# earthspecies/avex

Measured on AMD Instinct MI355X. Metric: clips/s (10 s @ 16 kHz) embedding extraction, BEATs-base, higher is better.
Workload: dtype f16; 1 GPU; BEATs-base (12L/768/3072/12H, 90.7 M params, synthetic weights), batch 256 x 10 s @ 16 kHz per GPU, wav resident in HBM -> mean-pooled 768-d embedding; global_batch=256, samples_per_clip=160000, parallelism=dp1, world_size=1, inputs=avex_amd.synth.noise_clips(seed=0), keyed by global clip index, chunk_clips=256, streams=1, residual_stream=half, layernorm_fold=True

## Files before the change

### avex_amd/_capi.py

```python
from __future__ import annotations

import ctypes as C
import os
from typing import Optional

HERE = os.path.dirname(os.path.abspath(__file__))
LIB_PATH = os.environ.get("AVEX_AMD_LIB") or os.path.join(HERE, "lib", "libavexhip.so")

F16, BF16 = 0, 1
DTYPE_NAMES = {"f16": F16, "fp16": F16, "float16": F16, "bf16": BF16, "bfloat16": BF16}


class AvexHipError(RuntimeError):
    """Raised for any failure of the HIP extension (missing library, no GPU, bad arguments)."""


class FbankConfig(C.Structure):
    _fields_ = [("win_length", C.c_int32), ("hop_length", C.c_int32), ("n_mels", C.c_int32),
                ("input_scale", C.c_float), ("preemph", C.c_float), ("remove_dc", C.c_int32),
                ("log_floor", C.c_float), ("norm_mean", C.c_float), ("norm_div", C.c_float)]


class MelspecConfig(C.Structure):
    _fields_ = [("n_fft", C.c_int32), ("hop_length", C.c_int32), ("win_length", C.c_int32), ("n_mels", C.c_int32),
# ... 126 lines not shown
    "avexhip_fbank_forward_padded": (C.c_int, [_P, _P, C.c_int, C.c_int64, C.c_int64, _P, C.c_int, _P, _P]),
    "avexhip_fbank_forward_patches": (C.c_int, [_P, _P, C.c_int, C.c_int64, C.c_int64, _P, C.c_int, C.c_int, _P, C.c_int, _P]),
    "avexhip_token_embed_ln": (C.c_int, [_P, _P, _P, _P, _P, C.c_float, C.c_int, C.c_int, C.c_int, _P, _P, C.c_int, _P]),
    "avexhip_cast_f32_to_half": (C.c_int, [_P, _P, C.c_int64, C.c_int, _P]),
    "avexhip_cast_half_to_f32": (C.c_int, [_P, _P, C.c_int64, C.c_int, _P]),
    "avexhip_gemm": (C.c_int, [C.POINTER(GemmArgs), C.c_int, _P]),
    "avexhip_pool_reduce": (C.c_int, [_P, C.c_int, C.c_int, C.c_int, _P, C.c_int64, _P]),
    "avexhip_pool_reduce_mode": (C.c_int, [_P, C.c_int, C.c_int, C.c_int, _P, C.c_int64, C.c_int, _P]),
    "avexhip_ln_rowstats": (C.c_int, [_P, C.c_int, C.c_int, C.c_float, _P, _P]),
    "avexhip_layernorm": (C.c_int, [_P, _P, C.c_int64, _P, _P, C.c_float, C.c_int, C.c_int, _P, C.c_int64, _P,
                                    C.c_int64, C.c_int, _P]),
    "avexhip_attention": (C.c_int, [_P, C.c_int, C.c_int, C.c_int, _P, _P, _P, _P, _P, _P, C.c_int, _P]),
    "avexhip_attention_hd": (C.c_int, [_P, C.c_int, C.c_int, C.c_int, C.c_int, _P, _P, C.c_int, _P]),
    "avexhip_posconv_pack": (C.c_int, [_P, _P, C.c_int, C.c_int, C.c_int, _P, C.c_int, _P]),
    "avexhip_posconv": (C.c_int, [_P, _P, _P, _P, C.c_int, C.c_int, C.c_int, C.c_int, C.c_int, _P, _P, C.c_int, _P]),
    "avexhip_mean_pool": (C.c_int, [_P, C.c_int, C.c_int, C.c_int, _P, _P]),
    "avexhip_rel_bucket": (C.c_int, [C.c_int, C.c_int, C.c_int]),
    "avexhip_beats_create": (_P, [C.POINTER(BeatsConfig), C.POINTER(Tensor), C.c_int]),
    "avexhip_beats_destroy": (None, [_P]),
    "avexhip_beats_num_tokens": (C.c_int, [_P, C.c_int64]),
    "avexhip_beats_workspace_bytes": (C.c_size_t, [_P, C.c_int, C.c_int64]),
    "avexhip_beats_forward": (C.c_int, [_P, _P, C.c_int, C.c_int64, C.c_int64, _P, C.c_uint32, C.POINTER(_P),
                                        C.c_int, _P, _P, _P, C.c_size_t, _P]),
    "avexhip_beats_forward_fbank": (C.c_int, [_P, _P, C.c_int, C.c_int, _P, C.c_uint32, C.POINTER(_P), C.c_int,
                                              _P, _P, _P, C.c_size_t, _P]),
    "avexhip_beats_graph_capture": (_P, [_P, _P, C.c_int, C.c_int64, C.c_int64, _P, C.c_uint32, C.POINTER(_P),
                                         C.c_int, _P, _P, _P, C.c_size_t, _P]),
    "avexhip_beats_graph_launch": (C.c_int, [_P, _P]),
    "avexhip_beats_graph_nodes": (C.c_int, [_P]),
    "avexhip_beats_graph_destroy": (None, [_P]),
# ... 131 lines not shown
```

### avex_amd/csrc/api.cpp

```cpp
#include <math.h>
#include <stdarg.h>
#include <stdlib.h>

#include <map>
#include <mutex>
#include <utility>
#include <string>
#include <vector>

#include "common.h"
#include "handle_core.h"

static thread_local char g_err[1024] = "";

void avexhip_set_error(const char* fmt, ...) {
    va_list ap;
    va_start(ap, fmt);
    vsnprintf(g_err, sizeof(g_err), fmt, ap);
    va_end(ap);
}

extern "C" const char* avexhip_last_error(void) { return g_err; }
extern "C" int avexhip_abi_version(void) { return AVEXHIP_ABI_VERSION; }
extern "C" int avexhip_device_count(void) {
// ... 75 lines not shown
extern "C" int avexhip_layernorm(const float* in, const void* in_half, int64_t ld_in, const float* w, const float* b,
                                 float eps, int M, int C, float* out_f32, int64_t ldo, void* out_half, int64_t ldh,
                                 int dtype, void* stream) {
    return avx::layernorm(in, in_half, ld_in, w, b, eps, M, C, out_f32, ldo, out_half, ldh, dtype, (hipStream_t)stream);
}

extern "C" int avexhip_attention(const void* qkv, int B, int T, int H, const float* bias_tab, const float* grep_w,
                                 const float* grep_b, const float* grep_a, const uint8_t* key_pad, void* out,
                                 int dtype, void* stream) {
    return avx::attention(qkv, B, T, H, bias_tab, grep_w, grep_b, grep_a, key_pad, out, dtype, (hipStream_t)stream);
}

extern "C" int avexhip_posconv_pack(const float* g, const float* v, int E, int groups, int K, void* w_packed,
                                    int dtype, void* stream) {
    return avx::posconv_pack(g, v, E, groups, K, w_packed, dtype, (hipStream_t)stream);
}

extern "C" int avexhip_posconv(const void* x_half, const float* x_f32, const void* w_packed, const float* bias, int B,
                               int T, int E, int groups, int K, float* out_f32, void* out_half, int dtype, void* stream) {
    return avx::posconv(x_half, x_f32, w_packed, bias, B, T, E, groups, K, out_f32, out_half, dtype, (hipStream_t)stream);
}

extern "C" int avexhip_token_embed_ln(const void* patches_half, const float* pos, const float* cls, const float* ln_w, const float* ln_b, float eps,
                                      int B, int n_patches, int C, void* out_half, float* out_f32, int dtype, void* stream) {
    return avx::token_embed_ln(patches_half, pos, cls, ln_w, ln_b, eps, B, n_patches, C, out_half, out_f32, dtype, (hipStream_t)stream);
}

extern "C" int avexhip_mean_pool(const float* in, int B, int T, int C, float* out, void* stream) {
    return avx::mean_pool(in, B, T, C, nullptr, out, (hipStream_t)stream);
}
// ... 80 lines not shown
    float* lnE_w = nullptr; float* lnE_b = nullptr;
    std::vector<Layer> layers;
    std::vector<float> rel_table;
    struct BiasTab { float* ptr; hipEvent_t ready; hipStream_t stream; bool done; };
    float* d_rel_table = nullptr;
    int* d_bucket_lut = nullptr;
    int lut_maxd = 0;
    char* bias_arena = nullptr; size_t bias_arena_bytes = 0, bias_arena_used = 0;
    std::map<int, BiasTab> bias_tabs;
    std::mutex bias_mu;

    CoreCfg core() const {
        CoreCfg c;
        c.E = E; c.F = F; c.H = H; c.L = L; c.alpha = alpha; c.eps = 1e-5f; c.hook_site = 0; c.fast = fast; c.fold = ln_fold;
        c.fold_min_rows = ln_fold_min_rows; c.batch_invariant = batch_invariant; c.act = act; c.glu = glu; c.hidden_shift = hidden_shift; c.pre_ln = pre_ln; c.final_ln_w = lnE_w; c.final_ln_b = lnE_b;
        return c;
    }
    ~avexhip_beats() override {
        for (auto& kv : bias_tabs) if (kv.second.ready) (void)hipEventDestroy(kv.second.ready);
        if (bias_arena) (void)hipFree(bias_arena);
        if (d_rel_table) (void)hipFree(d_rel_table);
        if (d_bucket_lut) (void)hipFree(d_bucket_lut);
        if (fb) avexhip_fbank_plan_destroy(fb);
        for (int i = 0; i < 3; ++i) { if (side[i]) (void)hipStreamDestroy(side[i]); if (ev_join[i]) (void)hipEventDestroy(ev_join[i]); }
        if (ev_fork) (void)hipEventDestroy(ev_fork);
    }
};

namespace {

const avxh::LayerNames BEATS_NAMES = {nullptr, "encoder.layers.%d.self_attn.q_proj", "encoder.layers.%d.self_attn.k_proj", "encoder.layers.%d.self_attn.v_proj",
                                      "encoder.layers.%d.self_attn.out_proj", "encoder.layers.%d.self_attn_layer_norm", "encoder.layers.%d.fc1",
// ... 244 lines not shown
        const int lane_id = li;
        hipStream_t cs = lane_id == 0 ? s : h->side[lane_id - 1];
        const Ws w = carve(h, (char*)workspace + (size_t)lane_id * need.total, chunk, Tt);
        const uint8_t* pad = frame_pad ? frame_pad + (size_t)c0 * Tt : nullptr;
        const double Md = (double)M;
        if (h->fe_in_lane) RC(frontend(c0, Bc, w, cs));

        const bool fast = h->fast;
        float* x32 = w.core.x;
        float* pre32 = fast ? nullptr : w.core.pre;
        void* preh = fast ? w.core.preh : nullptr;
        const bool hook0 = (hook_mask & 1u) != 0;
        avx::GemmArgs g;
        memset(&g, 0, sizeof(g)); g.ovf = h->d_ovf;
        g.A = w.patches; g.lda = P * P; g.W = h->w_patch; g.ldw = P * P; g.M = M; g.N = D; g.K = P * P; g.bias = h->b_patch;
        if (fast) { g.out_half = w.h0; g.ldh = D; } else { g.out_f32 = w.f0; g.ldo = D; }
        prof.begin("gemm.patch_embed", 2.0 * Md * D * P * P);
        RC(avx::gemm(g, dt, cs));
        prof.end();
        prof.begin("layernorm", 0.0);
        if (h->w_post) {
            RC(avx::layernorm(fast ? nullptr : w.f0, fast ? w.h0 : nullptr, D, h->ln0_w, h->ln0_b, 1e-5f, M, D, nullptr, D, w.h0, D, dt, cs));
        } else {
            RC(avx::layernorm(fast ? nullptr : w.f0, fast ? w.h0 : nullptr, D, h->ln0_w, h->ln0_b, 1e-5f, M, D, fast ? nullptr : x32, E, w.core.xh, E, dt, cs));
            RC(avx::zero_rows(fast ? nullptr : x32, E, w.core.xh, E, M, E, pad, cs));
        }
        prof.end();
        if (h->w_post) {
            memset(&g, 0, sizeof(g)); g.ovf = h->d_ovf;
            g.A = w.h0; g.lda = D; g.W = h->w_post; g.ldw = D; g.M = M; g.N = E; g.K = D; g.bias = h->b_post;
            g.out_half = w.core.xh; g.ldh = E; g.row_zero = pad;
            if (!fast || hook0) { g.out_f32 = x32; g.ldo = E; }
            prof.begin("gemm.post_extract_proj", 2.0 * Md * E * D);
            RC(avx::gemm(g, dt, cs));
            prof.end();
        }
        if (hook0 && h->w_post) {
            if (hook_pooled) RC(avx::agg_pool(x32, Bc, Tt, E, hook_pooled, hook_out[0] + (size_t)c0 * E, cs));
            else AVX_HIP_CHECK(hipMemcpyAsync(hook_out[0] + (size_t)c0 * Tt * E, x32, sizeof(float) * (size_t)M * E, hipMemcpyDeviceToDevice, cs));
        }
        prof.begin("posconv", 2.0 * Md * E * (E / h->cfg.conv_pos_groups) * h->cfg.conv_pos);
        RC(avx::posconv(w.core.xh, fast ? nullptr : x32, h->w_pc, h->b_pc, Bc, Tt, E, h->cfg.conv_pos_groups, h->cfg.conv_pos, pre32, preh, dt, cs));
        prof.end();
        if (!h->pre_ln) {
            prof.begin("layernorm", 0.0);
            RC(avx::layernorm(pre32, preh, E, h->lnE_w, h->lnE_b, 1e-5f, M, E, fast ? nullptr : x32, E, w.core.xh, E, dt, cs));
            prof.end();
        }

        CoreIo io;
        io.Bc = Bc; io.Tt = Tt; io.c0 = (size_t)c0; io.bias_tab = bias_tab; io.pad = pad; io.hook_mask = hook_mask; io.hook_bit0 = 1;
        io.hook_out = hook_out; io.hook_pooled = hook_pooled; io.features_out = features_out; io.pooled_out = pooled_out;
        RC(avxh::run_layers(h, h->core(), h->layers, w.core, io, prof, cs));
        if (L == 0) {
            if (features_out || pooled_out) {
                float* xo = features_out ? features_out + (size_t)c0 * Tt * E : x32;
                RC(avx::layernorm(pre32, preh, E, h->lnE_w, h->lnE_b, 1e-5f, M, E, xo, E, nullptr, E, dt, cs));
                if (pooled_out) RC(avx::mean_pool(xo, Bc, Tt, E, nullptr, pooled_out + (size_t)c0 * E, cs));
            }
        }
    }
    if (lanes > 1) {
        for (int i = 0; i + 1 < lanes; ++i) {
            if (h->ev_join[i]) (void)hipEventDestroy(h->ev_join[i]);
            AVX_HIP_CHECK(hipEventCreateWithFlags(&h->ev_join[i], hipEventDisableTiming));
            AVX_HIP_CHECK(hipEventRecord(h->ev_join[i], h->side[i]));
            AVX_HIP_CHECK(hipStreamWaitEvent(s, h->ev_join[i], 0));
// ... 244 lines not shown
```

### avex_amd/csrc/common.h

```cpp
#pragma once
#include <hip/hip_runtime.h>
#include <stdint.h>
#include <stdio.h>
#include <string.h>

#include "../../include/avexhip.h"

typedef _Float16 f16x8 __attribute__((ext_vector_type(8)));
typedef _Float16 f16x4 __attribute__((ext_vector_type(4)));
typedef __bf16 bf16x8 __attribute__((ext_vector_type(8)));
typedef __bf16 bf16x4 __attribute__((ext_vector_type(4)));
typedef float f32x4 __attribute__((ext_vector_type(4)));
typedef float f32x16 __attribute__((ext_vector_type(16)));

template <typename T> struct Half;
template <> struct Half<_Float16> {
    typedef f16x8 v8;
    typedef f16x4 v4;
    static __device__ __forceinline__ _Float16 from(float x) {
        const float lo = x < -65504.0f ? -65504.0f : x;
        return (_Float16)(lo > 65504.0f ? 65504.0f : lo);
    }
    static __device__ __forceinline__ _Float16 from_hw(float x) { return (_Float16)x; }
};
// ... 279 lines not shown
int gemm(const GemmArgs& a, int dtype, hipStream_t s);
int nhwc_to_nchw(const float* in, int64_t ld, int B, int HW, int C, const float* scale, const float* shift, float* out, hipStream_t s);
int64_t mbconv_front_tiles(int H, int W, int k, int stride, int kin);
int dwconv_parts(const void* in, int B, int H, int W, int Cp, int k, int stride, const float* w, const float* bias, void* out, float* part, size_t part_bytes,
                 int64_t* rows, int dtype, hipStream_t s);
int64_t dwconv_lds_tiles(int H, int W, int k, int stride);
int dwconv_lds_parts(const void* in, int B, int H, int W, int Cp, int k, int stride, const float* w, const float* bias, void* out, float* part,
                     size_t part_bytes, int64_t* rows, int dtype, hipStream_t s);
int se_from_parts(const float* part, int64_t rows, int B, int64_t hw, int C, int Cp, int Cs, const float* w1, const float* b1, const float* w2t,
                  const float* b2, float* scale, void* x, int dtype, hipStream_t s);
int mbconv_front(const void* in, int B, int H, int W, int ld_in, int kin, const void* w_exp, int ldw, const float* b_exp, int k, int stride,
                 const float* w_dw, const float* b_dw, int cp_exp, void* out, float* pool, float* part, size_t part_bytes, unsigned int* ovf,
                 int dtype, hipStream_t s);
int pool_reduce(const float* part, int B, int T, int N, float* out, int64_t ldo, hipStream_t s, int mode = 0);
int agg_pool(const float* in, int B, int T, int C, int mode, float* out, hipStream_t s);
int ln_rowstats(const float* stats, int M, int nseg, float eps, float* rows, hipStream_t s);
int bias_toeplitz(const float* rel_table, const int* lut, int maxd, int T, int H, float* out, hipStream_t s);
int lnr_fold(const float* gamma, const float* beta, const float* bias, float alpha, int N, float* ga, float* bb, hipStream_t s);
int layernorm(const float* in, const void* in_half, int64_t ld_in, const float* w, const float* b, float eps, int M,
              int C, float* out_f32, int64_t ldo, void* out_half, int64_t ldh, int dtype, hipStream_t s);
int cast_to_half(const float* in, void* out, int64_t n, int dtype, hipStream_t s, unsigned int* ovf = nullptr);
int row_sum_half(const void* w, int N, int K, float* out, int dtype, hipStream_t s);
int cast_to_f32(const void* in, float* out, int64_t n, int dtype, hipStream_t s);
int mean_pool(const float* in, int B, int T, int C, const uint8_t* frame_pad, float* out, hipStream_t s);
int token_embed_ln(const void* patches, const float* pos, const float* cls, const float* w, const float* b, float eps, int B, int Tp, int C,
                   void* out_half, float* out_f32, int dtype, hipStream_t s);
int glu_swish(const void* in, int64_t M, int F, void* out, unsigned int* ovf, int dtype, hipStream_t s);
int zero_rows(float* x32, int64_t ld32, void* x_half, int64_t ldh, int M, int C, const uint8_t* pad, hipStream_t s);
int layernorm_pool(const void* in_half, int64_t ld_in, const float* w, const float* b, float eps, int B, int T, int C, float* out, int dtype,
                   hipStream_t s);
bool gemm_streams(int M, int N);
bool gemm_post_ln_ok(const GemmArgs& a);
int attention(const void* qkv, int B, int T, int H, const float* bias_tab, const float* grep_w,
              const float* grep_b, const float* grep_a, const uint8_t* key_pad, void* out, int dtype,
              hipStream_t s, int q_log2e = 0);
int attention16(const void* qkv, int B, int T, int H, const float* bias_tab, const float* grep_w, const float* grep_b, const float* grep_a,
                const uint8_t* key_pad, void* out, int dtype, int q_log2e, int n_wg, hipStream_t s);
int attention_hd(const void* qkv, int B, int T, int H, int head_dim, const uint8_t* key_pad, void* out, int dtype, hipStream_t s, int q_log2e = 0);
int posconv_pack(const float* g, const float* v, int E, int groups, int K, void* w_packed, int dtype,
                 hipStream_t s);
int posconv(const void* x_half, const float* x_f32, const void* w_packed, const float* bias, int B, int T,
            int E, int groups, int K, float* out_f32, void* out_half, int dtype, hipStream_t s);

struct FbankDev {
    int win, hop, n_mels;
    float input_scale, preemph, log_floor, norm_mean, norm_div;
    int remove_dc;
    const float* window;
    const float2* twiddle;
    const int* mel_start;
    const int* mel_len;
    const int* mel_off;
    const float* mel_w;
};
int fbank(const FbankDev& fb, const float* wav, int B, int64_t T, int64_t stride, int frames,
          float* out_f32, void* out_patch, int patch, int dtype, hipStream_t s, const float* clip_offset = nullptr,
          int out_frames = 0);
// ... 5 lines not shown
```

### avex_amd/csrc/elementwise.hip

```cpp
#include "common.h"

namespace {

template <typename T>
__global__ void cast_to_half_kernel(const float* __restrict__ in, T* __restrict__ out, int64_t n, unsigned int* __restrict__ ovf) {
    int64_t i = ((int64_t)blockIdx.x * blockDim.x + threadIdx.x) * 4;
    const int64_t stride = (int64_t)gridDim.x * blockDim.x * 4;
    float ovf_mx = 0.f;
    for (; i + 3 < n; i += stride) {
        const f32x4 v = *(const f32x4*)(in + i);
        ovf_see4<T>(ovf_mx, v);
        typename Half<T>::v4 h;
        h[0] = Half<T>::from(v[0]); h[1] = Half<T>::from(v[1]);
        h[2] = Half<T>::from(v[2]); h[3] = Half<T>::from(v[3]);
        *(typename Half<T>::v4*)(out + i) = h;
    }
    if (blockIdx.x == 0 && threadIdx.x < (n & 3)) {
        const int64_t j = (n & ~(int64_t)3) + threadIdx.x;
        ovf_see<T>(ovf_mx, in[j], 0.f);
        out[j] = Half<T>::from(in[j]);
    }
    ovf_commit<T>(ovf, ovf_mx);
}

// ... 354 lines not shown
        *(v8*)(out + m * F + f) = o;
    }
    ovf_commit<T>(ovf, mx);
}

template <typename T>
__global__ __launch_bounds__(256) void row_sum_half_kernel(const T* __restrict__ w, int N, int K, float* __restrict__ out) {
    const int row = blockIdx.x * 4 + (threadIdx.x >> 6), lane = threadIdx.x & 63;
    if (row >= N) return;
    float s = 0.f;
    for (int k = lane; k < K; k += 64) s += (float)w[(int64_t)row * K + k];
    s = wave_sum(s);
    if (lane == 0) out[row] = s;
}

__global__ __launch_bounds__(256) void ln_rowstats_kernel(const float* __restrict__ stats, int M, int nseg, float eps, float* __restrict__ rows) {
    const int m = blockIdx.x * 256 + threadIdx.x;
    if (m >= M) return;
    const f32x4* src = (const f32x4*)(stats + (int64_t)m * nseg * 2);
    float s1 = 0.f, s2 = 0.f;
    for (int q = 0; q < (nseg >> 1); ++q) { const f32x4 v = src[q]; s1 += v[0] + v[2]; s2 += v[1] + v[3]; }
    const float inv = 1.0f / (float)(64 * nseg);
    const float mu = s1 * inv;
    const float var = fmaxf(__builtin_fmaf(-mu, mu, s2 * inv), 0.f);
    const float rstd = __builtin_amdgcn_rsqf(var + eps);
    ((float2*)rows)[m] = make_float2(rstd, -mu * rstd);
}

__global__ __launch_bounds__(256) void pool_reduce_kernel(const float* __restrict__ part, int B, int T, int N, float* __restrict__ out, int64_t ldo, int mode) {
    const int n = blockIdx.x * 256 + threadIdx.x, b = blockIdx.y;
    if (n >= N) return;
    const int64_t r0 = (int64_t)b * T, r1 = r0 + T - 1;
    float acc = mode == 1 ? -__builtin_inff() : 0.f;
    for (int64_t rb = r0 >> 6; rb <= (r1 >> 6); ++rb) {
        const int64_t first_clip = (rb * 64) / T;
        const float v = part[(rb * 2 + (first_clip == b ? 0 : 1)) * N + n];
        acc = mode == 1 ? fmaxf(acc, v) : acc + v;
// ... 37 lines not shown

int bias_toeplitz(const float* rel_table, const int* lut, int maxd, int T, int H, float* out, hipStream_t s) {
    const int n = H * (2 * T - 1);
    hipLaunchKernelGGL(bias_toeplitz_kernel, dim3((unsigned)((n + 255) / 256)), dim3(256), 0, s, rel_table, lut, maxd, T, H, out);
    AVX_LAUNCH_CHECK();
    return AVEXHIP_OK;
}

int lnr_fold(const float* gamma, const float* beta, const float* bias, float alpha, int N, float* ga, float* bb, hipStream_t s) {
    AVX_REQUIRE(gamma && beta && bias && ga && bb && N > 0, "lnr_fold: bad arguments");
    hipLaunchKernelGGL(lnr_fold_kernel, dim3((N + 255) / 256), dim3(256), 0, s, gamma, beta, bias, alpha, N, ga, bb);
    AVX_LAUNCH_CHECK();
    return AVEXHIP_OK;
}

int ln_rowstats(const float* stats, int M, int nseg, float eps, float* rows, hipStream_t s) {
    AVX_REQUIRE(stats && rows && M > 0, "ln_rowstats: bad arguments");
    AVX_REQUIRE(nseg > 0 && nseg % 2 == 0, "ln_rowstats: nseg = %d (row width must be a multiple of 128)", nseg);
    hipLaunchKernelGGL(ln_rowstats_kernel, dim3((M + 255) / 256), dim3(256), 0, s, stats, M, nseg, eps, rows);
    AVX_LAUNCH_CHECK();
    return AVEXHIP_OK;
}

int row_sum_half(const void* w, int N, int K, float* out, int dtype, hipStream_t s) {
    AVX_REQUIRE(w && out && N > 0 && K > 0, "row_sum_half: bad arguments");
    if (dtype == AVEXHIP_BF16) hipLaunchKernelGGL(row_sum_half_kernel<__bf16>, dim3((N + 3) / 4), dim3(256), 0, s, (const __bf16*)w, N, K, out);
    else hipLaunchKernelGGL(row_sum_half_kernel<_Float16>, dim3((N + 3) / 4), dim3(256), 0, s, (const _Float16*)w, N, K, out);
    AVX_LAUNCH_CHECK();
    return AVEXHIP_OK;
}


int cast_to_half(const float* in, void* out, int64_t n, int dtype, hipStream_t s, unsigned int* ovf) {
    AVX_REQUIRE(in && out && n >= 0, "cast_to_half: bad arguments");
// ... 171 lines not shown
```

### avex_amd/csrc/handle_core.h

```cpp
#pragma once
#include <math.h>
#include <stdlib.h>

#include <map>
#include <string>
#include <vector>

#include "common.h"

namespace avxh {

inline size_t align_up(size_t x, size_t a = 256) { return (x + a - 1) / a * a; }

struct StageRec {
    std::string name;
    double flops;
    hipEvent_t e0, e1;
};

struct HandleBase {
    int dtype = AVEXHIP_F16;
    const char* who = "create";
    std::vector<void*> allocs;
    unsigned int* d_ovf = nullptr;
// ... 247 lines not shown

struct CoreCfg {
    int E = 0, F = 0, H = 0, L = 0;
    int head_dim = 64;
    float alpha = 1.f, eps = 1e-5f;
    int hook_site = 0;
    bool fast = false;
    bool fold = false;
    int fold_min_rows = 0;
    int act = 1;
    bool glu = false;
    int hidden_shift = 0;
    bool pre_ln = false;
    bool batch_invariant = false;
    const float* final_ln_w = nullptr; const float* final_ln_b = nullptr;
};

inline bool cfg_fast(int residual_dtype) { return (residual_dtype & 1) != 0; }
inline bool cfg_batch_invariant(int residual_dtype) {
    const char* e = getenv("AVEX_AMD_BATCH_INVARIANT");
    return (residual_dtype & 2) != 0 || (e && atoi(e) != 0);
}
inline void fold_policy(bool fast, int E, int F, bool* fold, int* min_rows, bool batch_invariant = false) {
    const char* e = getenv("AVEX_AMD_LN_FOLD");
    const bool is_auto = !e || e[0] == 'a' || e[0] == 'A';
    *fold = fast && E % 256 == 0 && F % 256 == 0 && !(e && !is_auto && atoi(e) == 0);
    int rows = 4096;
    if (e && is_auto) { const char* c = strchr(e, ':'); if (c && atoi(c + 1) > 0) rows = atoi(c + 1); }
    *min_rows = is_auto && !batch_invariant ? rows : 0;
}
// ... 58 lines not shown
    RC(dev_f32(h, tb, fmt_name(nm.ln2, i, ".weight"), E, &ly.ln2_w));
    RC(dev_f32(h, tb, fmt_name(nm.ln2, i, ".bias"), E, &ly.ln2_b));
    if (c.fold) {
        auto two = [&](float** ga, float** bb) -> int {
            AVX_HIP_CHECK(hipMalloc((void**)ga, sizeof(float) * 2 * (size_t)E));
            h->allocs.push_back(*ga);
            *bb = *ga + E;
            return AVEXHIP_OK;
        };
        RC(two(&ly.ga_fc2, &ly.bb_fc2));
        RC(avx::lnr_fold(ly.ln1_w, ly.ln1_b, ly.b_fc2, c.alpha, E, ly.ga_fc2, ly.bb_fc2, nullptr));
        std::vector<float> Wh, bh;
        RC(host_f32(h, tb, fmt_name(nm.fc1, i, ".weight"), (int64_t)F * E, Wh));
        RC(host_f32(h, tb, fmt_name(nm.fc1, i, ".bias"), F, bh));
        RC(fold_ln(h, Wh, bh, F, E, ly.ln1_w, ly.ln1_b, &ly.w_fc1_f, &ly.b_fc1_f, &ly.s_fc1));
        if (i > 0) {
            const Layer& prev = layers[i - 1];
            RC(two(&ly.ga_o, &ly.bb_o));
            RC(avx::lnr_fold(prev.ln2_w, prev.ln2_b, ly.b_o, c.alpha, E, ly.ga_o, ly.bb_o, nullptr));
            RC(fold_ln(h, Wqkv, bqkv, 3 * E, E, prev.ln2_w, prev.ln2_b, &ly.w_qkv_f, &ly.b_qkv_f, &ly.s_qkv));
        }
    }
#undef RC
    return AVEXHIP_OK;
}

struct CoreWs {
    float* x; char* xh; float* pre; char* preh; char* qkv; char* ah; char* hh; float* raw;
    char* hh2;
    float* pool;
    float* splitk; size_t splitk_bytes;
    float* st1; float* st2;
    float* r1; float* r2;
};

// ... 19 lines not shown
    return w;
}

struct CoreIo {
    int Bc = 0, Tt = 0;
    size_t c0 = 0;
    const float* bias_tab = nullptr;
    const uint8_t* pad = nullptr;
    uint32_t hook_mask = 0;
    int hook_bit0 = 0;
    float* const* hook_out = nullptr;
    int hook_pooled = 0;
    float* features_out = nullptr;
    float* pooled_out = nullptr;
    float* final_f32 = nullptr;
};

struct Tap {
    bool hooked = false, fused = false;
    float* out = nullptr;
};
inline Tap tap_begin(const CoreCfg& c, const CoreWs& w, const CoreIo& io, int layer, avx::GemmArgs& g) {
    Tap t;
    t.hooked = (io.hook_mask >> (io.hook_bit0 + layer)) & 1u;
    if (!t.hooked) return t;
    const size_t per_clip = io.hook_pooled ? (size_t)c.E : (size_t)io.Tt * c.E;
    t.out = io.hook_out[io.hook_bit0 + layer] + io.c0 * per_clip;
    static const bool no_fuse = getenv("AVEX_AMD_POOL_FUSE") && atoi(getenv("AVEX_AMD_POOL_FUSE")) == 0;
    const bool streams = g.ln_rows || g.lnr_y || g.stats_out || avx::gemm_streams(g.M, g.N);
    t.fused = io.hook_pooled && io.Tt >= 64 && c.E % 256 == 0 && g.K >= 128 && streams && !no_fuse && !(c.batch_invariant && io.hook_pooled == 1);
    if (t.fused) {
// ... 110 lines not shown
#undef RC
    return AVEXHIP_OK;
}

inline int run_layers(HandleBase* h, const CoreCfg& c, const std::vector<Layer>& layers, const CoreWs& w, CoreIo& io, Prof& prof, hipStream_t cs) {
    const int E = c.E, F = c.F, H = c.H, L = c.L, dt = h->dtype, Bc = io.Bc, Tt = io.Tt;
    const int M = Bc * Tt;
    const double Md = (double)M;
    const bool fast = c.fast;
    if (c.pre_ln) return run_layers_pre_ln(h, c, layers, w, io, prof, cs);
    float* x32 = w.x;
    float* pre32 = fast ? nullptr : w.pre;
    void* preh = fast ? w.preh : nullptr;
    int rc;
#define RC(x) do { rc = (x); if (rc != AVEXHIP_OK) return rc; } while (0)
    const bool fold = fast && c.fold && F > 0 && M >= c.fold_min_rows;
    const int nseg = E / 64;
    avx::GemmArgs g;
    io.final_f32 = nullptr;
    for (int i = 0; i < L; ++i) {
        const Layer& ly = layers[i];
        const bool raw_in = fold && i > 0;
        memset(&g, 0, sizeof(g)); g.ovf = h->d_ovf;
        g.A = w.xh; g.lda = E; g.W = ly.w_qkv; g.ldw = E; g.M = M; g.N = 3 * E; g.K = E; g.bias = ly.b_qkv;
        g.out_half = w.qkv; g.ldh = 3 * E;
        if (raw_in) { g.W = ly.w_qkv_f; g.bias = ly.b_qkv_f; g.ln_rows = w.r2; g.ln_s = ly.s_qkv; }
        prof.begin("gemm.qkv", 2.0 * Md * 3 * E * E);
        pin_kernel(c, g); RC(avx::gemm(g, dt, cs));
        prof.end();
        prof.begin("attention", 4.0 * Md * Tt * E + (ly.grep_w ? 2.0 * Md * 8 * (E / H) * H : 0.0));
        RC(self_attention(h, c, ly, w, io, cs));
        prof.end();
        memset(&g, 0, sizeof(g)); g.ovf = h->d_ovf;
        g.A = w.ah; g.lda = E; g.W = ly.w_o; g.ldw = E; g.M = M; g.N = E; g.K = E; g.bias = ly.b_o; g.alpha = c.alpha;
        if (fast) { g.resid_half = w.xh; g.ldrh = E; g.out_half = preh; g.ldh = E; }
        else { g.resid = x32; g.ldr = E; g.out_f32 = pre32; g.ldo = E; }
        if (fold) {
// ... 107 lines not shown
```

### avex_amd/csrc/posconv.hip

```cpp
#include "common.h"

namespace {

constexpr int CG = 48;
constexpr int KT = 128;
constexpr int PAD = KT / 2;
constexpr int TMAX = 512;
constexpr int SLAB_ROWS = TMAX + KT;
constexpr int SLAB_BYTES = SLAB_ROWS * CG * 2;
constexpr int KTOT = KT * CG;
constexpr int NU = KT / 2;
constexpr int WST = CG * 96 * 2;
constexpr int PC_LDS = SLAB_BYTES + 2 * WST;

static __device__ __forceinline__ void pc_dma16(const void* src, const char* lds_dst) {
    const unsigned lds = (unsigned)(__UINTPTR_TYPE__)(__attribute__((address_space(3))) const char*)lds_dst;
    asm volatile("s_mov_b32 m0, %1\n\tglobal_load_lds_dwordx4 %0, off" ::"v"(src), "s"(lds) : "memory");
}

template <typename T>
__global__ __launch_bounds__(512) __attribute__((amdgpu_waves_per_eu(4, 4)))
void posconv_kernel(const T* __restrict__ xh, const float* __restrict__ xf, const T* __restrict__ wp,
                    const float* __restrict__ bias, int Tn, int E, int G, int nseg, float* __restrict__ out, T* __restrict__ out_h) {
    extern __shared__ __attribute__((aligned(16))) char slab[];
    typedef typename Half<T>::v8 v8;
    char* wring = slab + SLAB_BYTES;
    const int tid = threadIdx.x, lane = tid & 63;
    const int wave = __builtin_amdgcn_readfirstlane(tid >> 6);
    const int g = blockIdx.x % G, bs = blockIdx.x / G;
    const int b = bs / nseg, t0 = (bs - b * nseg) * TMAX;
    const T* xg = xh + (int64_t)b * Tn * E + g * CG;
    const char* wg = (const char*)(wp + (int64_t)g * CG * KTOT);

    auto issue_w = [&](int u) __attribute__((always_inline)) {
        const char* src = wg + (int64_t)u * WST;
        char* dst = wring + (u & 1) * WST;
        pc_dma16(src + wave * 1024 + lane * 16, dst + wave * 1024);
        if (wave == (u & 7)) pc_dma16(src + 8 * 1024 + lane * 16, dst + 8 * 1024);
// ... 44 lines not shown
#pragma unroll
                for (int ot = 0; ot < 3; ++ot)
#pragma unroll
                    for (int tt = 0; tt < 4; ++tt) acc[ot][tt] = mfma16(wf[ot], xfr[tt], acc[ot][tt]);
            }
        }
        asm volatile("s_waitcnt vmcnt(0) lgkmcnt(0)" ::: "memory");
        __builtin_amdgcn_s_barrier();
    }
    if (!has_work) return;

    AVX_F16_SAT_BEGIN();
#pragma unroll
    for (int tt = 0; tt < 4; ++tt) {
        const int tl = tw0 + tt * 16 + t16, t = t0 + tl;
        if (t >= Tn) continue;
        const int64_t rowoff = ((int64_t)b * Tn + t) * E + g * CG;
#pragma unroll
        for (int ot = 0; ot < 3; ++ot) {
            const int n = ot * 16 + 4 * g4;
            f32x4 v = acc[ot][tt] + *(const f32x4*)(bias + g * CG + n);
            v = gelu_erf4(v);
            f32x4 r;
            if (xf) {
                r = *(const f32x4*)(xf + rowoff + n);
            } else {
                const typename Half<T>::v4 rh = *(const typename Half<T>::v4*)(slab + (tl + PAD) * (CG * 2) + n * 2);
                r = (f32x4){(float)rh[0], (float)rh[1], (float)rh[2], (float)rh[3]};
            }
            r += v;
            if (out) *(f32x4*)(out + rowoff + n) = r;
            if (out_h) {
                typename Half<T>::v4 h;
                h[0] = Half<T>::from_hw(r[0]); h[1] = Half<T>::from_hw(r[1]);
                h[2] = Half<T>::from_hw(r[2]); h[3] = Half<T>::from_hw(r[3]);
                *(typename Half<T>::v4*)(out_h + rowoff + n) = h;
            }
        }
    }
}

__global__ __launch_bounds__(256) void posconv_norm_kernel(const float* __restrict__ v, int n_rows, int K,
                                                           float* __restrict__ norm) {
    __shared__ float red[4];
    const int k = blockIdx.x;
    float s = 0.f;
    for (int r = threadIdx.x; r < n_rows; r += 256) {
        const float x = v[(int64_t)r * K + k];
        s += x * x;
    }
    s = wave_sum(s);
    if ((threadIdx.x & 63) == 0) red[threadIdx.x >> 6] = s;
// ... 33 lines not shown
    const dim3 grid((unsigned)((total + 255) / 256));
    if (dtype == AVEXHIP_BF16)
        hipLaunchKernelGGL(posconv_pack_kernel<__bf16>, grid, dim3(256), 0, s, v, g, norm, E, cg, K, (__bf16*)w_packed);
    else
        hipLaunchKernelGGL(posconv_pack_kernel<_Float16>, grid, dim3(256), 0, s, v, g, norm, E, cg, K, (_Float16*)w_packed);
    hipError_t e = hipGetLastError();
    hipError_t e2 = hipStreamSynchronize(s);
    (void)hipFree(norm);
    if (e != hipSuccess || e2 != hipSuccess) {
        avexhip_set_error("posconv_pack: %s", hipGetErrorString(e != hipSuccess ? e : e2));
        return AVEXHIP_ERR_HIP;
    }
    return AVEXHIP_OK;
}

int posconv(const void* x_half, const float* x_f32, const void* w_packed, const float* bias, int B, int T,
            int E, int groups, int K, float* out, void* out_half, int dtype, hipStream_t s) {
    AVX_REQUIRE(x_half && w_packed && bias && (out || out_half), "posconv: null argument");
    AVX_REQUIRE(groups > 0 && E % groups == 0 && E / groups == CG && K == KT,
                "posconv: only %d channels/group and %d taps are built (got E=%d groups=%d K=%d)", CG, KT, E, groups, K);
    AVX_REQUIRE(B > 0 && T > 0, "posconv: empty input B=%d T=%d", B, T);
    const int nseg = (T + TMAX - 1) / TMAX;
    if (dtype == AVEXHIP_BF16) {
        AVX_ENSURE_LDS(posconv_kernel<__bf16>, PC_LDS);
        hipLaunchKernelGGL(posconv_kernel<__bf16>, dim3(B * nseg * groups), dim3(512), PC_LDS, s, (const __bf16*)x_half, x_f32,
                           (const __bf16*)w_packed, bias, T, E, groups, nseg, out, (__bf16*)out_half);
    } else if (dtype == AVEXHIP_F16) {
        AVX_ENSURE_LDS(posconv_kernel<_Float16>, PC_LDS);
        hipLaunchKernelGGL(posconv_kernel<_Float16>, dim3(B * nseg * groups), dim3(512), PC_LDS, s, (const _Float16*)x_half, x_f32,
                           (const _Float16*)w_packed, bias, T, E, groups, nseg, out, (_Float16*)out_half);
    } else {
        avexhip_set_error("posconv: unknown dtype %d", dtype);
        return AVEXHIP_ERR_INVALID;
    }
    AVX_LAUNCH_CHECK();
    return AVEXHIP_OK;
}

}
```

### avex_amd/kernels.py

```python
from __future__ import annotations

import ctypes as C
import logging
import math
import os
import warnings
from typing import Dict, List, Mapping, Optional, Sequence, Tuple

import numpy as np
import torch

from . import _capi
from ._capi import AvexHipError, BeatsConfig, FbankConfig, GemmArgs, MelspecConfig, Tensor, check, dtype_code, lib

logger = logging.getLogger(__name__)

F32_EPS = 1.1920929e-07


def _stream() -> int:
    return int(torch.cuda.current_stream().cuda_stream)


def _ptr(t: Optional[torch.Tensor]) -> Optional[int]:
# ... 496 lines not shown


def posconv(x_half: torch.Tensor, x_f32: Optional[torch.Tensor], w_packed: torch.Tensor, bias: torch.Tensor,
            groups: int, K: int = 128, half_out: bool = False) -> torch.Tensor:
    _need_cuda(x_half, w_packed, bias)
    code = _capi.F16 if x_half.dtype == torch.float16 else _capi.BF16
    B, T, E = x_half.shape
    x_half = x_half.contiguous()
    out = torch.empty((B, T, E), dtype=x_half.dtype if half_out else torch.float32, device=x_half.device)
    check(lib().avexhip_posconv(_ptr(x_half), None if x_f32 is None else _ptr(x_f32.contiguous()), _ptr(w_packed),
                                _ptr(bias), B, T, E, groups, K, None if half_out else _ptr(out),
                                _ptr(out) if half_out else None, code, _stream()), "posconv")
    return out


def token_embed_ln(patches: torch.Tensor, pos: torch.Tensor, cls: torch.Tensor, ln_w: torch.Tensor, ln_b: torch.Tensor, eps: float,
                   B: int, want_f32: bool = False) -> Tuple[torch.Tensor, Optional[torch.Tensor]]:
    _need_cuda(patches, pos, cls, ln_w, ln_b)
    code = _capi.F16 if patches.dtype == torch.float16 else _capi.BF16
    M, Cc = patches.shape
    n = M // B
    outh = torch.empty((B * (n + 1), Cc), dtype=patches.dtype, device=patches.device)
    outf = torch.empty((B * (n + 1), Cc), dtype=torch.float32, device=patches.device) if want_f32 else None
    check(lib().avexhip_token_embed_ln(_ptr(patches.contiguous()), _ptr(pos.contiguous()), _ptr(cls.contiguous()), _ptr(ln_w), _ptr(ln_b), eps,
                                       B, n, Cc, _ptr(outh), _ptr(outf), code, _stream()), "token_embed_ln")
    return outh, outf


def mean_pool(x: torch.Tensor) -> torch.Tensor:
    _need_cuda(x)
# ... 333 lines not shown
```

### include/avexhip.h

```cpp
#ifndef AVEXHIP_H
#define AVEXHIP_H

#include <stddef.h>
#include <stdint.h>

#ifdef __cplusplus
extern "C" {
#endif

#define AVEXHIP_ABI_VERSION 13

enum { AVEXHIP_F16 = 0, AVEXHIP_BF16 = 1 };

enum {
    AVEXHIP_OK = 0,
    AVEXHIP_ERR_INVALID = -1,
    AVEXHIP_ERR_HIP = -2,
    AVEXHIP_ERR_MISSING = -3,
    AVEXHIP_ERR_WORKSPACE = -4
};

const char* avexhip_last_error(void);
int avexhip_abi_version(void);
int avexhip_device_count(void);
// ... 132 lines not shown
                      const float* bias, float eps, int M, int C, float* out_f32, int64_t ldo,
                      void* out_half, int64_t ldh, int dtype, void* stream);

int avexhip_attention(const void* qkv_dev, int B, int T, int H, const float* bias_tab,
                      const float* grep_w, const float* grep_b, const float* grep_a,
                      const uint8_t* key_pad, void* out_dev, int dtype, void* stream);

int avexhip_attention_hd(const void* qkv_dev, int B, int T, int H, int head_dim, const uint8_t* key_pad, void* out_dev, int dtype,
                         void* stream);

int avexhip_posconv_pack(const float* g_dev, const float* v_dev, int E, int groups, int K,
                         void* w_packed_dev, int dtype, void* stream);
int avexhip_posconv(const void* x_half_dev, const float* x_f32_dev, const void* w_packed_dev,
                    const float* bias_dev, int B, int T, int E, int groups, int K,
                    float* out_f32_dev, void* out_half_dev, int dtype, void* stream);

int avexhip_token_embed_ln(const void* patches_half, const float* pos, const float* cls, const float* ln_w, const float* ln_b, float eps,
                           int B, int n_patches, int C, void* out_half, float* out_f32, int dtype, void* stream);

int avexhip_mean_pool(const float* in_dev, int B, int T, int C, float* out_dev, void* stream);

#ifdef AVEX_DIAG
int avexhip_debug_lds_canary(int blocks, int iters, unsigned* report_dev, void* stream);
int avexhip_debug_gemm_stamps(int enable, unsigned long long* host_out, int n_blocks);
int avexhip_debug_gemm_clocks(unsigned long long* host_out, int n_tiles);
int avexhip_debug_gemm_kclocks(unsigned long long* host_out, int n_blocks);
#endif

typedef struct {
    const float* query;
// ... 269 lines not shown
```

Baseline: 10170 clips/s.

## Fold front-end LayerNorm into layer-0 QKV via posconv-emitted row stats

```diff
diff --git a/avex_amd/_capi.py b/avex_amd/_capi.py
--- a/avex_amd/_capi.py
+++ b/avex_amd/_capi.py
@@ -164,6 +164,7 @@
     "avexhip_attention_hd": (C.c_int, [_P, C.c_int, C.c_int, C.c_int, C.c_int, _P, _P, C.c_int, _P]),
     "avexhip_posconv_pack": (C.c_int, [_P, _P, C.c_int, C.c_int, C.c_int, _P, C.c_int, _P]),
     "avexhip_posconv": (C.c_int, [_P, _P, _P, _P, C.c_int, C.c_int, C.c_int, C.c_int, C.c_int, _P, _P, C.c_int, _P]),
+    "avexhip_posconv_stats": (C.c_int, [_P, _P, _P, C.c_int, C.c_int, C.c_int, C.c_int, C.c_int, _P, _P, _P, C.c_float, C.c_int, _P]),
     "avexhip_mean_pool": (C.c_int, [_P, C.c_int, C.c_int, C.c_int, _P, _P]),
     "avexhip_rel_bucket": (C.c_int, [C.c_int, C.c_int, C.c_int]),
     "avexhip_beats_create": (_P, [C.POINTER(BeatsConfig), C.POINTER(Tensor), C.c_int]),
diff --git a/avex_amd/csrc/api.cpp b/avex_amd/csrc/api.cpp
--- a/avex_amd/csrc/api.cpp
+++ b/avex_amd/csrc/api.cpp
@@ -113,6 +113,14 @@
 extern "C" int avexhip_posconv_pack(const float* g, const float* v, int E, int groups, int K, void* w_packed,
                                     int dtype, void* stream) {
     return avx::posconv_pack(g, v, E, groups, K, w_packed, dtype, (hipStream_t)stream);
+}
+
+extern "C" int avexhip_posconv_stats(const void* x_half, const void* w_packed, const float* bias, int B, int T, int E, int groups, int K,
+                                     void* out_half, float* stats_out, float* rows_out, float eps, int dtype, void* stream) {
+    const int rc = avx::posconv(x_half, nullptr, w_packed, bias, B, T, E, groups, K, nullptr, out_half, dtype, (hipStream_t)stream, stats_out);
+    if (rc != AVEXHIP_OK || !rows_out) return rc;
+    AVX_REQUIRE(stats_out, "posconv_stats: rows_out needs stats_out");
+    return avx::ln_rowstats(stats_out, B * T, groups, eps, rows_out, (hipStream_t)stream, E / groups, true);
 }
 
 extern "C" int avexhip_posconv(const void* x_half, const float* x_f32, const void* w_packed, const float* bias, int B,
@@ -223,8 +231,10 @@
         CoreCfg c;
         c.E = E; c.F = F; c.H = H; c.L = L; c.alpha = alpha; c.eps = 1e-5f; c.hook_site = 0; c.fast = fast; c.fold = ln_fold;
         c.fold_min_rows = ln_fold_min_rows; c.batch_invariant = batch_invariant; c.act = act; c.glu = glu; c.hidden_shift = hidden_shift; c.pre_ln = pre_ln; c.final_ln_w = lnE_w; c.final_ln_b = lnE_b;
+        if (front_fold()) { c.in_ln_w = lnE_w; c.in_ln_b = lnE_b; }
         return c;
     }
+    bool front_fold() const { return fast && ln_fold && !pre_ln && w_post && L > 0 && F > 0; }
     ~avexhip_beats() override {
         for (auto& kv : bias_tabs) if (kv.second.ready) (void)hipEventDestroy(kv.second.ready);
         if (bias_arena) (void)hipFree(bias_arena);
@@ -499,6 +509,7 @@
         avx::GemmArgs g;
         memset(&g, 0, sizeof(g)); g.ovf = h->d_ovf;
         g.A = w.patches; g.lda = P * P; g.W = h->w_patch; g.ldw = P * P; g.M = M; g.N = D; g.K = P * P; g.bias = h->b_patch;
+        const bool front = h->front_fold() && avxh::folds(h->core(), M) && M >= 2;
         if (fast) { g.out_half = w.h0; g.ldh = D; } else { g.out_f32 = w.f0; g.ldo = D; }
         prof.begin("gemm.patch_embed", 2.0 * Md * D * P * P);
         RC(avx::gemm(g, dt, cs));
@@ -511,10 +522,11 @@
             RC(avx::zero_rows(fast ? nullptr : x32, E, w.core.xh, E, M, E, pad, cs));
         }
         prof.end();
+        char* xin = front ? w.core.hh : w.core.xh;
         if (h->w_post) {
             memset(&g, 0, sizeof(g)); g.ovf = h->d_ovf;
             g.A = w.h0; g.lda = D; g.W = h->w_post; g.ldw = D; g.M = M; g.N = E; g.K = D; g.bias = h->b_post;
-            g.out_half = w.core.xh; g.ldh = E; g.row_zero = pad;
+            g.out_half = xin; g.ldh = E; g.row_zero = pad;
             if (!fast || hook0) { g.out_f32 = x32; g.ldo = E; }
             prof.begin("gemm.post_extract_proj", 2.0 * Md * E * D);
             RC(avx::gemm(g, dt, cs));
@@ -524,10 +536,16 @@
             if (hook_pooled) RC(avx::agg_pool(x32, Bc, Tt, E, hook_pooled, hook_out[0] + (size_t)c0 * E, cs));
             else AVX_HIP_CHECK(hipMemcpyAsync(hook_out[0] + (size_t)c0 * Tt * E, x32, sizeof(float) * (size_t)M * E, hipMemcpyDeviceToDevice, cs));
         }
-        prof.begin("posconv", 2.0 * Md * E * (E / h->cfg.conv_pos_groups) * h->cfg.conv_pos);
-        RC(avx::posconv(w.core.xh, fast ? nullptr : x32, h->w_pc, h->b_pc, Bc, Tt, E, h->cfg.conv_pos_groups, h->cfg.conv_pos, pre32, preh, dt, cs));
+        const int G = h->cfg.conv_pos_groups;
+        prof.begin("posconv", 2.0 * Md * E * (E / G) * h->cfg.conv_pos);
+        if (front) RC(avx::posconv(xin, nullptr, h->w_pc, h->b_pc, Bc, Tt, E, G, h->cfg.conv_pos, nullptr, w.core.xh, dt, cs, (float*)w.core.qkv));
+        else RC(avx::posconv(w.core.xh, fast ? nullptr : x32, h->w_pc, h->b_pc, Bc, Tt, E, G, h->cfg.conv_pos, pre32, preh, dt, cs));
         prof.end();
-        if (!h->pre_ln) {
+        if (front) {
+            prof.begin("ln_rowstats", 0.0);
+            RC(avx::ln_rowstats((const float*)w.core.qkv, M, G, 1e-5f, w.core.r2, cs, E / G, true));
+            prof.end();
+        } else if (!h->pre_ln) {
             prof.begin("layernorm", 0.0);
             RC(avx::layernorm(pre32, preh, E, h->lnE_w, h->lnE_b, 1e-5f, M, E, fast ? nullptr : x32, E, w.core.xh, E, dt, cs));
             prof.end();
@@ -536,6 +554,7 @@
         CoreIo io;
         io.Bc = Bc; io.Tt = Tt; io.c0 = (size_t)c0; io.bias_tab = bias_tab; io.pad = pad; io.hook_mask = hook_mask; io.hook_bit0 = 1;
         io.hook_out = hook_out; io.hook_pooled = hook_pooled; io.features_out = features_out; io.pooled_out = pooled_out;
+        io.raw_in = front;
         RC(avxh::run_layers(h, h->core(), h->layers, w.core, io, prof, cs));
         if (L == 0) {
             if (features_out || pooled_out) {
diff --git a/avex_amd/csrc/common.h b/avex_amd/csrc/common.h
--- a/avex_amd/csrc/common.h
+++ b/avex_amd/csrc/common.h
@@ -317,7 +317,7 @@
                  int dtype, hipStream_t s);
 int pool_reduce(const float* part, int B, int T, int N, float* out, int64_t ldo, hipStream_t s, int mode = 0);
 int agg_pool(const float* in, int B, int T, int C, int mode, float* out, hipStream_t s);
-int ln_rowstats(const float* stats, int M, int nseg, float eps, float* rows, hipStream_t s);
+int ln_rowstats(const float* stats, int M, int nseg, float eps, float* rows, hipStream_t s, int seg_width = 64, bool planes = false);
 int bias_toeplitz(const float* rel_table, const int* lut, int maxd, int T, int H, float* out, hipStream_t s);
 int lnr_fold(const float* gamma, const float* beta, const float* bias, float alpha, int N, float* ga, float* bb, hipStream_t s);
 int layernorm(const float* in, const void* in_half, int64_t ld_in, const float* w, const float* b, float eps, int M,
@@ -343,7 +343,7 @@
 int posconv_pack(const float* g, const float* v, int E, int groups, int K, void* w_packed, int dtype,
                  hipStream_t s);
 int posconv(const void* x_half, const float* x_f32, const void* w_packed, const float* bias, int B, int T,
-            int E, int groups, int K, float* out_f32, void* out_half, int dtype, hipStream_t s);
+            int E, int groups, int K, float* out_f32, void* out_half, int dtype, hipStream_t s, float* stats_out = nullptr);
 
 struct FbankDev {
     int win, hop, n_mels;
diff --git a/avex_amd/csrc/elementwise.hip b/avex_amd/csrc/elementwise.hip
--- a/avex_amd/csrc/elementwise.hip
+++ b/avex_amd/csrc/elementwise.hip
@@ -392,13 +392,28 @@
     if (lane == 0) out[row] = s;
 }
 
-__global__ __launch_bounds__(256) void ln_rowstats_kernel(const float* __restrict__ stats, int M, int nseg, float eps, float* __restrict__ rows) {
+__global__ __launch_bounds__(256) void ln_rowstats_kernel(const float* __restrict__ stats, int M, int nseg, int width, float eps, float* __restrict__ rows) {
     const int m = blockIdx.x * 256 + threadIdx.x;
     if (m >= M) return;
     const f32x4* src = (const f32x4*)(stats + (int64_t)m * nseg * 2);
     float s1 = 0.f, s2 = 0.f;
     for (int q = 0; q < (nseg >> 1); ++q) { const f32x4 v = src[q]; s1 += v[0] + v[2]; s2 += v[1] + v[3]; }
-    const float inv = 1.0f / (float)(64 * nseg);
+    const float inv = 1.0f / (float)(width * nseg);
+    const float mu = s1 * inv;
+    const float var = fmaxf(__builtin_fmaf(-mu, mu, s2 * inv), 0.f);
+    const float rstd = __builtin_amdgcn_rsqf(var + eps);
+    ((float2*)rows)[m] = make_float2(rstd, -mu * rstd);
+}
+
+__global__ __launch_bounds__(256) void ln_rowstats_planes_kernel(const float2* __restrict__ stats, int M, int nseg, int width, float eps, float* __restrict__ rows) {
+    const int m = blockIdx.x * 256 + threadIdx.x;
+    if (m >= M) return;
+    float s1 = 0.f, s2 = 0.f;
+    for (int q = 0; q < nseg; q += 2) {
+        const float2 a = stats[(int64_t)q * M + m], b = stats[(int64_t)(q + 1) * M + m];
+        s1 += a.x + b.x; s2 += a.y + b.y;
+    }
+    const float inv = 1.0f / (float)(width * nseg);
     const float mu = s1 * inv;
     const float var = fmaxf(__builtin_fmaf(-mu, mu, s2 * inv), 0.f);
     const float rstd = __builtin_amdgcn_rsqf(var + eps);
@@ -466,10 +481,11 @@
     return AVEXHIP_OK;
 }
 
-int ln_rowstats(const float* stats, int M, int nseg, float eps, float* rows, hipStream_t s) {
-    AVX_REQUIRE(stats && rows && M > 0, "ln_rowstats: bad arguments");
-    AVX_REQUIRE(nseg > 0 && nseg % 2 == 0, "ln_rowstats: nseg = %d (row width must be a multiple of 128)", nseg);
-    hipLaunchKernelGGL(ln_rowstats_kernel, dim3((M + 255) / 256), dim3(256), 0, s, stats, M, nseg, eps, rows);
+int ln_rowstats(const float* stats, int M, int nseg, float eps, float* rows, hipStream_t s, int seg_width, bool planes) {
+    AVX_REQUIRE(stats && rows && M > 0 && seg_width > 0, "ln_rowstats: bad arguments");
+    AVX_REQUIRE(nseg > 0 && nseg % 2 == 0, "ln_rowstats: nseg = %d (an even number of segments)", nseg);
+    if (planes) hipLaunchKernelGGL(ln_rowstats_planes_kernel, dim3((M + 255) / 256), dim3(256), 0, s, (const float2*)stats, M, nseg, seg_width, eps, rows);
+    else hipLaunchKernelGGL(ln_rowstats_kernel, dim3((M + 255) / 256), dim3(256), 0, s, stats, M, nseg, seg_width, eps, rows);
     AVX_LAUNCH_CHECK();
     return AVEXHIP_OK;
 }
diff --git a/avex_amd/csrc/handle_core.h b/avex_amd/csrc/handle_core.h
--- a/avex_amd/csrc/handle_core.h
+++ b/avex_amd/csrc/handle_core.h
@@ -285,6 +285,7 @@
     bool pre_ln = false;
     bool batch_invariant = false;
     const float* final_ln_w = nullptr; const float* final_ln_b = nullptr;
+    const float* in_ln_w = nullptr; const float* in_ln_b = nullptr;
 };
 
 inline bool cfg_fast(int residual_dtype) { return (residual_dtype & 1) != 0; }
@@ -373,11 +374,12 @@
         RC(host_f32(h, tb, fmt_name(nm.fc1, i, ".weight"), (int64_t)F * E, Wh));
         RC(host_f32(h, tb, fmt_name(nm.fc1, i, ".bias"), F, bh));
         RC(fold_ln(h, Wh, bh, F, E, ly.ln1_w, ly.ln1_b, &ly.w_fc1_f, &ly.b_fc1_f, &ly.s_fc1));
-        if (i > 0) {
-            const Layer& prev = layers[i - 1];
+        if (i > 0 || c.in_ln_w) {
+            const float* pw = i > 0 ? layers[i - 1].ln2_w : c.in_ln_w;
+            const float* pb = i > 0 ? layers[i - 1].ln2_b : c.in_ln_b;
             RC(two(&ly.ga_o, &ly.bb_o));
-            RC(avx::lnr_fold(prev.ln2_w, prev.ln2_b, ly.b_o, c.alpha, E, ly.ga_o, ly.bb_o, nullptr));
-            RC(fold_ln(h, Wqkv, bqkv, 3 * E, E, prev.ln2_w, prev.ln2_b, &ly.w_qkv_f, &ly.b_qkv_f, &ly.s_qkv));
+            RC(avx::lnr_fold(pw, pb, ly.b_o, c.alpha, E, ly.ga_o, ly.bb_o, nullptr));
+            RC(fold_ln(h, Wqkv, bqkv, 3 * E, E, pw, pb, &ly.w_qkv_f, &ly.b_qkv_f, &ly.s_qkv));
         }
     }
 #undef RC
@@ -427,7 +429,10 @@
     float* features_out = nullptr;
     float* pooled_out = nullptr;
     float* final_f32 = nullptr;
-};
+    bool raw_in = false;
+};
+
+inline bool folds(const CoreCfg& c, int M) { return c.fast && c.fold && !c.pre_ln && c.F > 0 && M >= c.fold_min_rows; }
 
 struct Tap {
     bool hooked = false, fused = false;
@@ -568,13 +573,14 @@
     void* preh = fast ? w.preh : nullptr;
     int rc;
 #define RC(x) do { rc = (x); if (rc != AVEXHIP_OK) return rc; } while (0)
-    const bool fold = fast && c.fold && F > 0 && M >= c.fold_min_rows;
+    const bool fold = folds(c, M);
+    AVX_REQUIRE(!io.raw_in || (fold && c.in_ln_w), "run_layers: raw input without a folded LayerNorm in front of layer 0");
     const int nseg = E / 64;
     avx::GemmArgs g;
     io.final_f32 = nullptr;
     for (int i = 0; i < L; ++i) {
         const Layer& ly = layers[i];
-        const bool raw_in = fold && i > 0;
+        const bool raw_in = fold && (i > 0 || io.raw_in);
         memset(&g, 0, sizeof(g)); g.ovf = h->d_ovf;
         g.A = w.xh; g.lda = E; g.W = ly.w_qkv; g.ldw = E; g.M = M; g.N = 3 * E; g.K = E; g.bias = ly.b_qkv;
         g.out_half = w.qkv; g.ldh = 3 * E;
diff --git a/avex_amd/csrc/posconv.hip b/avex_amd/csrc/posconv.hip
--- a/avex_amd/csrc/posconv.hip
+++ b/avex_amd/csrc/posconv.hip
@@ -18,10 +18,11 @@
     asm volatile("s_mov_b32 m0, %1\n\tglobal_load_lds_dwordx4 %0, off" ::"v"(src), "s"(lds) : "memory");
 }
 
-template <typename T>
+template <typename T, bool STATS>
 __global__ __launch_bounds__(512) __attribute__((amdgpu_waves_per_eu(4, 4)))
 void posconv_kernel(const T* __restrict__ xh, const float* __restrict__ xf, const T* __restrict__ wp,
-                    const float* __restrict__ bias, int Tn, int E, int G, int nseg, float* __restrict__ out, T* __restrict__ out_h) {
+                    const float* __restrict__ bias, int Tn, int E, int G, int nseg, float* __restrict__ out, T* __restrict__ out_h,
+                    float* __restrict__ stats) {
     extern __shared__ __attribute__((aligned(16))) char slab[];
     typedef typename Half<T>::v8 v8;
     char* wring = slab + SLAB_BYTES;
@@ -96,28 +97,41 @@
 #pragma unroll
     for (int tt = 0; tt < 4; ++tt) {
         const int tl = tw0 + tt * 16 + t16, t = t0 + tl;
-        if (t >= Tn) continue;
+        const bool live = t < Tn;
         const int64_t rowoff = ((int64_t)b * Tn + t) * E + g * CG;
-#pragma unroll
-        for (int ot = 0; ot < 3; ++ot) {
-            const int n = ot * 16 + 4 * g4;
-            f32x4 v = acc[ot][tt] + *(const f32x4*)(bias + g * CG + n);
-            v = gelu_erf4(v);
-            f32x4 r;
-            if (xf) {
-                r = *(const f32x4*)(xf + rowoff + n);
-            } else {
-                const typename Half<T>::v4 rh = *(const typename Half<T>::v4*)(slab + (tl + PAD) * (CG * 2) + n * 2);
-                r = (f32x4){(float)rh[0], (float)rh[1], (float)rh[2], (float)rh[3]};
+        float s1 = 0.f, s2 = 0.f;
+        if (live) {
+#pragma unroll
+            for (int ot = 0; ot < 3; ++ot) {
+                const int n = ot * 16 + 4 * g4;
+                f32x4 v = acc[ot][tt] + *(const f32x4*)(bias + g * CG + n);
+                v = gelu_erf4(v);
+                f32x4 r;
+                if (xf) {
+                    r = *(const f32x4*)(xf + rowoff + n);
+                } else {
+                    const typename Half<T>::v4 rh = *(const typename Half<T>::v4*)(slab + (tl + PAD) * (CG * 2) + n * 2);
+                    r = (f32x4){(float)rh[0], (float)rh[1], (float)rh[2], (float)rh[3]};
+                }
+                r += v;
+                if (out) *(f32x4*)(out + rowoff + n) = r;
+                if (out_h) {
+                    typename Half<T>::v4 h;
+                    h[0] = Half<T>::from_hw(r[0]); h[1] = Half<T>::from_hw(r[1]);
+                    h[2] = Half<T>::from_hw(r[2]); h[3] = Half<T>::from_hw(r[3]);
+                    *(typename Half<T>::v4*)(out_h + rowoff + n) = h;
+                    if (STATS) {
+#pragma unroll
+                        for (int e = 0; e < 4; ++e) { const float q = (float)h[e]; s1 += q; s2 = __builtin_fmaf(q, q, s2); }
+                    }
+                }
             }
-            r += v;
-            if (out) *(f32x4*)(out + rowoff + n) = r;
-            if (out_h) {
-                typename Half<T>::v4 h;
-                h[0] = Half<T>::from_hw(r[0]); h[1] = Half<T>::from_hw(r[1]);
-                h[2] = Half<T>::from_hw(r[2]); h[3] = Half<T>::from_hw(r[3]);
-                *(typename Half<T>::v4*)(out_h + rowoff + n) = h;
-            }
+        }
+        if (STATS) {
+            s1 += __shfl_xor(s1, 16, 64); s2 += __shfl_xor(s2, 16, 64);
+            s1 += __shfl_xor(s1, 32, 64); s2 += __shfl_xor(s2, 32, 64);
+            const int64_t Mtot = (int64_t)(gridDim.x / (G * nseg)) * Tn;
+            if (live && g4 == 0) *(float2*)(stats + (g * Mtot + (int64_t)b * Tn + t) * 2) = make_float2(s1, s2);
         }
     }
 }
@@ -181,25 +195,35 @@
     return AVEXHIP_OK;
 }
 
+template <typename T_, bool STATS>
+static int posconv_launch(const void* x_half, const float* x_f32, const void* w_packed, const float* bias, int B, int T, int E, int groups,
+                          float* out, void* out_half, float* stats, hipStream_t s) {
+    const int nseg = (T + TMAX - 1) / TMAX;
+    AVX_ENSURE_LDS((posconv_kernel<T_, STATS>), PC_LDS);
+    hipLaunchKernelGGL((posconv_kernel<T_, STATS>), dim3(B * nseg * groups), dim3(512), PC_LDS, s, (const T_*)x_half, x_f32, (const T_*)w_packed, bias,
+                       T, E, groups, nseg, out, (T_*)out_half, stats);
+    return AVEXHIP_OK;
+}
+
 int posconv(const void* x_half, const float* x_f32, const void* w_packed, const float* bias, int B, int T,
-            int E, int groups, int K, float* out, void* out_half, int dtype, hipStream_t s) {
+            int E, int groups, int K, float* out, void* out_half, int dtype, hipStream_t s, float* stats_out) {
     AVX_REQUIRE(x_half && w_packed && bias && (out || out_half), "posconv: null argument");
     AVX_REQUIRE(groups > 0 && E % groups == 0 && E / groups == CG && K == KT,
                 "posconv: only %d channels/group and %d taps are built (got E=%d groups=%d K=%d)", CG, KT, E, groups, K);
     AVX_REQUIRE(B > 0 && T > 0, "posconv: empty input B=%d T=%d", B, T);
-    const int nseg = (T + TMAX - 1) / TMAX;
+    AVX_REQUIRE(!stats_out || (out_half && out_half != x_half), "posconv: stats_out are taken over the half output, which must not be the input");
+    int rc;
     if (dtype == AVEXHIP_BF16) {
-        AVX_ENSURE_LDS(posconv_kernel<__bf16>, PC_LDS);
-        hipLaunchKernelGGL(posconv_kernel<__bf16>, dim3(B * nseg * groups), dim3(512), PC_LDS, s, (const __bf16*)x_half, x_f32,
-                           (const __bf16*)w_packed, bias, T, E, groups, nseg, out, (__bf16*)out_half);
+        rc = stats_out ? posconv_launch<__bf16, true>(x_half, x_f32, w_packed, bias, B, T, E, groups, out, out_half, stats_out, s)
+                       : posconv_launch<__bf16, false>(x_half, x_f32, w_packed, bias, B, T, E, groups, out, out_half, nullptr, s);
     } else if (dtype == AVEXHIP_F16) {
-        AVX_ENSURE_LDS(posconv_kernel<_Float16>, PC_LDS);
-        hipLaunchKernelGGL(posconv_kernel<_Float16>, dim3(B * nseg * groups), dim3(512), PC_LDS, s, (const _Float16*)x_half, x_f32,
-                           (const _Float16*)w_packed, bias, T, E, groups, nseg, out, (_Float16*)out_half);
+        rc = stats_out ? posconv_launch<_Float16, true>(x_half, x_f32, w_packed, bias, B, T, E, groups, out, out_half, stats_out, s)
+                       : posconv_launch<_Float16, false>(x_half, x_f32, w_packed, bias, B, T, E, groups, out, out_half, nullptr, s);
     } else {
         avexhip_set_error("posconv: unknown dtype %d", dtype);
         return AVEXHIP_ERR_INVALID;
     }
+    if (rc != AVEXHIP_OK) return rc;
     AVX_LAUNCH_CHECK();
     return AVEXHIP_OK;
 }
diff --git a/avex_amd/kernels.py b/avex_amd/kernels.py
--- a/avex_amd/kernels.py
+++ b/avex_amd/kernels.py
@@ -534,6 +534,21 @@
     return out
 
 
+def posconv_stats(x_half: torch.Tensor, w_packed: torch.Tensor, bias: torch.Tensor, groups: int, K: int = 128,
+                  eps: float = 1e-5) -> Dict[str, torch.Tensor]:
+    _need_cuda(x_half, w_packed, bias)
+    code = _capi.F16 if x_half.dtype == torch.float16 else _capi.BF16
+    B, T, E = x_half.shape
+    x_half = x_half.contiguous()
+    M = B * T
+    out = torch.empty((B, T, E), dtype=x_half.dtype, device=x_half.device)
+    stats = torch.empty((groups, M, 2), dtype=torch.float32, device=x_half.device)
+    rows = torch.zeros((M + (M & 1), 2), dtype=torch.float32, device=x_half.device)
+    check(lib().avexhip_posconv_stats(_ptr(x_half), _ptr(w_packed), _ptr(bias), B, T, E, groups, K, _ptr(out), _ptr(stats), _ptr(rows),
+                                      float(eps), code, _stream()), "posconv_stats")
+    return {"out": out, "stats": stats, "rows": rows}
+
+
 def token_embed_ln(patches: torch.Tensor, pos: torch.Tensor, cls: torch.Tensor, ln_w: torch.Tensor, ln_b: torch.Tensor, eps: float,
                    B: int, want_f32: bool = False) -> Tuple[torch.Tensor, Optional[torch.Tensor]]:
     _need_cuda(patches, pos, cls, ln_w, ln_b)
diff --git a/include/avexhip.h b/include/avexhip.h
--- a/include/avexhip.h
+++ b/include/avexhip.h
@@ -170,6 +170,8 @@
 int avexhip_posconv(const void* x_half_dev, const float* x_f32_dev, const void* w_packed_dev,
                     const float* bias_dev, int B, int T, int E, int groups, int K,
                     float* out_f32_dev, void* out_half_dev, int dtype, void* stream);
+int avexhip_posconv_stats(const void* x_half_dev, const void* w_packed_dev, const float* bias_dev, int B, int T, int E, int groups, int K,
+                          void* out_half_dev, float* stats_out_dev, float* rows_out_dev, float eps, int dtype, void* stream);
 
 int avexhip_token_embed_ln(const void* patches_half, const float* pos, const float* cls, const float* ln_w, const float* ln_b, float eps,
                            int B, int n_patches, int C, void* out_half, float* out_f32, int dtype, void* stream);
```

After: 10200 clips/s, median of 6. No clear change (+0.2%).
